# GAP-LAB-CUHK-SZ/gaustudio

Measured on NVIDIA B200. Metric: views/sec fwd+bwd @1M Gaussians/1080p, higher is better.
Workload: dtype f32

## Files before the change

gaustudio_b200/_C.py:

```python
import ctypes as C
import threading

import torch

from . import _lib

_pipeline = threading.local()


def set_pipelined(enabled, slack=1.25, fixed_capacity=None):
    _pipeline.enabled = bool(enabled)
    _pipeline.fixed = int(fixed_capacity) if fixed_capacity else 0
    _pipeline.slack = float(slack)
    _pipeline.hw = {}
    _pipeline.pending = []
    _pipeline.ring = None
    _pipeline.slot = 0
    _pipeline.rmax = None


def _pl():
    if not hasattr(_pipeline, "enabled"):
        set_pipelined(False)
    return _pipeline
# ... 229 lines not shown
        radii = radii.contiguous()
        with _on_device(dev):
            stream = torch.cuda.current_stream(dev)
            rc = L.gsr_backward(P, int(degree), M, int(R), _ptr(background), W, H, _ptr(means3D), _ptr(sh),
                                _ptr(colors), _ptr(scales), float(scale_modifier), _ptr(rotations),
                                _ptr(cov3D_precomp), _ptr(viewmatrix), _ptr(projmatrix), _ptr(campos), float(tan_fovx),
                                float(tan_fovy), _ptr(radii), _ptr(geomBuffer), _ptr(binningBuffer),
                                _ptr(imageBuffer), _ptr(gc), _ptr(gd), _ptr(gm), _ptr(go), _ptr(dL_dmeans2D), None,
                                _ptr(dL_dopacity), _ptr(dL_dcolors), None, _ptr(dL_dmeans3D), _ptr(dL_dcov3D),
                                _ptr(dL_dsh), _ptr(dL_dscales), _ptr(dL_drotations), int(bool(debug)),
                                stream.cuda_stream)
        if rc < 0:
            raise RuntimeError("gsr_backward failed: " + _lib.last_error())
    return dL_dmeans2D, dL_dcolors, dL_dopacity, dL_dmeans3D, dL_dcov3D, dL_dsh, dL_dscales, dL_drotations


def rasterize_gaussians_fused_backward(background, means3D, radii, f_dc, f_rest, opacity_logits, log_scales,
                                       raw_rotations, scale_modifier, viewmatrix, projmatrix, tan_fovx, tan_fovy,
                                       dL_dout_color, dL_dout_depth, dL_dout_median_depth, dL_dout_final_opacity,
                                       degree, campos, geomBuffer, R, binningBuffer, imageBuffer, debug):
    L = _lib.lib()
    dev = means3D.device
    P = means3D.size(0)
    H, W = dL_dout_color.size(1), dL_dout_color.size(2)
    fopt = dict(dtype=torch.float32, device=dev)
    f_dc, f_rest = _f32(f_dc, dev, "f_dc"), _f32(f_rest, dev, "f_rest")
    M = 1 + (f_rest.numel() // (3 * P) if f_rest.numel() else 0)
    d_m3 = torch.empty(P, 3, **fopt); d_m2 = torch.empty(P, 3, **fopt); d_op = torch.empty_like(opacity_logits)
    d_dc = torch.empty_like(f_dc); d_rest = torch.empty_like(f_rest); d_sc = torch.empty(P, 3, **fopt)
    d_rot = torch.empty(P, 4, **fopt); d_col = torch.empty(P, 3, **fopt); d_cov = torch.empty(P, 6, **fopt)
    means3D = _f32(means3D, dev, "means3D"); opacity_logits = _f32(opacity_logits, dev, "opacity")
    log_scales = _f32(log_scales, dev, "scales"); raw_rotations = _f32(raw_rotations, dev, "rotations")
    viewmatrix = _f32(viewmatrix, dev, "viewmatrix"); projmatrix = _f32(projmatrix, dev, "projmatrix")
    campos = _f32(campos, dev, "campos"); background = _f32(_bg_on(background, dev), dev, "bg")
    gc = _f32(dL_dout_color, dev, "dL_dout_color"); gd = _f32(dL_dout_depth, dev, "dL_dout_depth")
    gm = _f32(dL_dout_median_depth, dev, "dL_dout_median_depth"); go = _f32(dL_dout_final_opacity, dev, "dL_dout_opacity")
    with _on_device(dev):
        stream = torch.cuda.current_stream(dev)
        rc = L.gsr_backward_fused(P, int(degree), M, int(R), _ptr(background), W, H, _ptr(means3D), _ptr(f_dc),
                                  _ptr(f_rest), _ptr(opacity_logits), _ptr(log_scales), float(scale_modifier),
                                  _ptr(raw_rotations), _ptr(viewmatrix), _ptr(projmatrix), _ptr(campos), float(tan_fovx),
                                  float(tan_fovy), _ptr(radii), _ptr(geomBuffer), _ptr(binningBuffer), _ptr(imageBuffer),
                                  _ptr(gc), _ptr(gd), _ptr(gm), _ptr(go), _ptr(d_m2), _ptr(d_op), _ptr(d_col), _ptr(d_m3),
                                  _ptr(d_cov), _ptr(d_dc), _ptr(d_rest), _ptr(d_sc), _ptr(d_rot), int(bool(debug)),
                                  stream.cuda_stream)
    if rc < 0:
        raise RuntimeError("gsr_backward_fused failed: " + _lib.last_error())
    return d_m2, d_op, d_m3, d_dc, d_rest, d_sc, d_rot


def mark_visible(means3D, viewmatrix, projmatrix):
    L = _lib.lib()
    dev = means3D.device
    P = means3D.size(0)
    present = torch.zeros(P, dtype=torch.bool, device=dev)
    if P != 0:
        means3D = _f32(means3D, dev, "means3D")
        viewmatrix = _f32(viewmatrix, dev, "viewmatrix"); projmatrix = _f32(projmatrix, dev, "projmatrix")
        with torch.cuda.device(dev):
            rc = L.gsr_mark_visible(P, _ptr(means3D), _ptr(viewmatrix), _ptr(projmatrix), present.data_ptr(),
                                    torch.cuda.current_stream(dev).cuda_stream)
        if rc < 0:
            raise RuntimeError("gsr_mark_visible failed: " + _lib.last_error())
    return present


def debug_export(P, W, H, R, geomBuffer, binningBuffer, imageBuffer):
# ... 23 lines not shown
```

gaustudio_b200/csrc/gsr_api.cu:

```cuda
#include "../../include/gsr.h"
#include "gsr_internal.cuh"
#include <cmath>

#include <cstdio>
#include <cstdlib>
#include <atomic>
#include <cstring>
#include <mutex>
#include <string>
#include <vector>

#include <cuda.h>
#include <nvtx3/nvToolsExt.h>

namespace gsr {

namespace {
thread_local std::string g_err;

inline size_t align_up(size_t v, size_t a) { return (v + a - 1) / a * a; }

template <typename T> inline void take(char*& p, T*& out, size_t count) {
  p = reinterpret_cast<char*>(align_up(reinterpret_cast<size_t>(p), 256));
  out = reinterpret_cast<T*>(p);
// ... 187 lines not shown
  int dev = -1;
  bool ready(int d) {
    if (dev == d && counts && ev) return true;
    if (ev) { cudaEventDestroy(ev); ev = nullptr; }
    if (!counts && cudaHostAlloc(reinterpret_cast<void**>(&counts), 16, cudaHostAllocDefault) != cudaSuccess) { counts = nullptr; cudaGetLastError(); return false; }
    if (cudaEventCreateWithFlags(&ev, cudaEventDisableTiming) != cudaSuccess) { ev = nullptr; cudaGetLastError(); return false; }
    dev = d;
    return true;
  }
};
thread_local SpecHost t_spec;
inline long long spec_capacity(long long binned) { return binned + binned / 4 + 4096; }

__global__ void k_set_capacity(ImageHeader* h, unsigned long long cap) {
  h->capacity = cap;
  h->overflow = 0;
  h->num_big = 0;
  h->ticket[0] = 0;
  h->ticket[1] = 0;
}

__global__ void k_depth2normal(const float* __restrict__ depth, int W, int H, float ifx, float ify, float ox, float oy,
                               float dmin, float dmax, const float* __restrict__ rot, float* __restrict__ out) {
  const int u = blockIdx.x * blockDim.x + threadIdx.x, v = blockIdx.y * blockDim.y + threadIdx.y;
  if (u >= W || v >= H) return;
  float* o = out + ((size_t)v * W + u) * 3;
  float n0 = -1.f, n1 = -1.f, n2 = -1.f, c0, c1, c2;
  if (cross_normal(depth, u, v, W, H, ifx, ify, ox, oy, dmin, dmax, c0, c1, c2)) {
    if (rot) {
      n0 = c0 * rot[0] + c1 * rot[3] + c2 * rot[6];
      n1 = c0 * rot[1] + c1 * rot[4] + c2 * rot[7];
      n2 = c0 * rot[2] + c1 * rot[5] + c2 * rot[8];
    } else {
      n0 = c0; n1 = c1; n2 = c2;
    }
  }
  o[0] = n0; o[1] = n1; o[2] = n2;
}

__global__ void k_depth2point(const float* __restrict__ depth, int W, int H, float ifx, float ify, float ox, float oy,
                              const float* __restrict__ c2w, float* __restrict__ out) {
  const int u = blockIdx.x * blockDim.x + threadIdx.x, v = blockIdx.y * blockDim.y + threadIdx.y;
  if (u >= W || v >= H) return;
  const float z = depth[(size_t)v * W + u];
  const float uz = __fmul_rn(__fmul_rn(__fdiv_rn((float)u, (float)(W - 1)), (float)(W - 1)), z);
  const float vz = __fmul_rn(__fmul_rn(__fdiv_rn((float)v, (float)(H - 1)), (float)(H - 1)), z);
  float x = __fadd_rn(__fmul_rn(uz, ifx), __fmul_rn(z, ox));
  float y = __fadd_rn(__fmul_rn(vz, ify), __fmul_rn(z, oy));
  float zz = z;
  if (c2w) {
    const float wx = c2w[0] * x + c2w[1] * y + c2w[2] * z + c2w[3];
// ... 17 lines not shown
  if (depths) depths[i] = q1.z;
  if (rgb) { rgb[3 * i] = q1.w; rgb[3 * i + 1] = q2.x; rgb[3 * i + 2] = q2.y; }
  if (cov3D) for (int k = 0; k < 6; k++) cov3D[6 * i + k] = vis ? g.cov3D[6 * i + k] : 0.f;
  if (tiles_touched) tiles_touched[i] = g.tiles_touched[i];
  if (clamped) { const unsigned char c = vis ? g.clamped[i] : 0; clamped[3 * i] = c & 1; clamped[3 * i + 1] = (c >> 1) & 1; clamped[3 * i + 2] = (c >> 2) & 1; }
}
__global__ void k_export_list(long long R, const ImageHeader* hdr, BinView b, uint32_t* point_list) {
  const long long i = (long long)blockIdx.x * blockDim.x + threadIdx.x;
  const long long binned = (long long)min(hdr->num_rendered, hdr->capacity);
  if (i < R) point_list[i] = i < binned ? b.point_list[i] : 0xffffffffu;
}
__global__ void k_export_image(int N, int T, ImageView im, uint32_t* ranges, uint32_t* n_contrib, float* final_T) {
  const int i = blockIdx.x * blockDim.x + threadIdx.x;
  if (i < N) {
    if (n_contrib) n_contrib[i] = im.n_contrib[i];
    if (final_T) final_T[i] = im.final_T[i];
  }
  if (i < T && ranges) { ranges[2 * i] = im.tile_range[i].x; ranges[2 * i + 1] = im.tile_range[i].y; }
}
}

void launch_depth2normal(const float* depth, int W, int H, float fx, float fy, float cx, float cy, float dmin,
                         float dmax, const float* rot, float* out, cudaStream_t st) {
  dim3 blk(32, 8), grd((W + 31) / 32, (H + 7) / 8);
  launch_high_priority(k_depth2normal, grd, blk, 0, st, depth, W, H, 1.0f / fx, 1.0f / fy, -cx / fx, -cy / fy, dmin, dmax, rot, out);
}

void launch_depth2point(const float* depth, int W, int H, float fx, float fy, float cx, float cy, const float* c2w,
                        float* out, cudaStream_t st) {
  dim3 blk(32, 8), grd((W + 31) / 32, (H + 7) / 8);
  k_depth2point<<<grd, blk, 0, st>>>(depth, W, H, 1.0f / fx, 1.0f / fy, -cx / fx, -cy / fy, c2w, out);
}

void launch_debug_export(int P, int W, int H, long long R, GeomView g, BinView b, ImageView im,
                         uint32_t* point_list, uint32_t* ranges, uint32_t* n_contrib, float* final_T,
                         float* means2D, float* conic_opacity, float* depths, float* rgb, float* cov3D,
                         uint32_t* tiles_touched, unsigned char* clamped, cudaStream_t st) {
  if (P > 0) k_export_geom<<<(P + 255) / 256, 256, 0, st>>>(P, g, means2D, conic_opacity, depths, rgb, cov3D, tiles_touched, clamped);
  if (R > 0 && point_list) k_export_list<<<(unsigned)((R + 255) / 256), 256, 0, st>>>(R, im.hdr, b, point_list);
  const int N = W * H, T = ((W + TILE_X - 1) / TILE_X) * ((H + TILE_Y - 1) / TILE_Y);
  k_export_image<<<(max(N, T) + 255) / 256, 256, 0, st>>>(N, T, im, ranges, n_contrib, final_T);
}

}

using namespace gsr;

// ... 103 lines not shown
    if (r_host) *r_host = counts[0];
    cap = counts[0];
    ret = counts[1];
    if (!dbg && cudaGetDevice(&dev) == cudaSuccess) hint_put(dev, P, width, height, cap);
  }
  if (!second_half(cap)) return -1;
  return ret;
}

static int backward_impl(int fused, const float* f_dc, const float* f_rest, const float* opacities_raw, float* dL_df_dc, float* dL_df_rest, int P, int D, int M, int64_t R, const float* background, int width, int height,
                 const float* means3D, const float* shs, const float* colors_precomp, const float* scales,
                 float scale_modifier, const float* rotations, const float* cov3D_precomp, const float* viewmatrix,
                 const float* projmatrix, const float* campos, float tan_fovx, float tan_fovy, const int* radii,
                 char* geom_buffer, char* binning_buffer, char* image_buffer, const float* dL_dpix,
                 const float* dL_dpix_depth, const float* dL_dpix_median_depth, const float* dL_dpix_final_opacity,
                 float* dL_dmean2D, float* dL_dconic, float* dL_dopacity, float* dL_dcolor, float* dL_ddepth,
                 float* dL_dmean3D, float* dL_dcov3D, float* dL_dsh, float* dL_dscale, float* dL_drot, int debug,
                 void* stream) {
  cudaStream_t st = (cudaStream_t)stream;
  const bool dbg = debug != 0;
  if (P <= 0) return 0;
  if (!geom_buffer || !image_buffer || (!binning_buffer && R > 0)) { g_err = "gsr_backward: missing state buffers"; return -1; }
  if (!background) { g_err = "gsr_backward: background must be a device pointer (backward.cu:586 reads it)"; return -1; }
  const int gx = (width + TILE_X - 1) / TILE_X, gy = (height + TILE_Y - 1) / TILE_Y;
  GeomView g = carve_geom(aligned_base(geom_buffer), P);
  ImageView im = carve_image(aligned_base(image_buffer), width, height);
  BinView b = carve_binning(aligned_base(binning_buffer), R);
  if (radii == nullptr) radii = g.radii;

  if (!check(cudaMemsetAsync(g.grad, 0, sizeof(float) * GRAD_F * (size_t)P, st), "memset grad")) return -1;
  if (R > 0) {
    { Prof pf(5, st); launch_render_bwd(width, height, gx, gy, background, im, b, g, dL_dpix, dL_dpix_depth, dL_dpix_median_depth,
                      dL_dpix_final_opacity, st); }
    if (!stage_ok(dbg, st, "render_bwd")) return -1;
  }
  BwdArgs a;
  a.P = P; a.D = D; a.M = M; a.W = width; a.H = height;
  a.means3D = means3D; a.shs = shs; a.colors_precomp = colors_precomp; a.scales = scales; a.rotations = rotations;
  a.cov3D_precomp = cov3D_precomp; a.view = viewmatrix; a.proj = projmatrix; a.campos = campos;
  a.scale_modifier = scale_modifier; a.tan_fovx = tan_fovx; a.tan_fovy = tan_fovy;
  a.focal_y = height / (2.0f * tan_fovy);
  a.focal_x = width / (2.0f * tan_fovx);
  a.radii = radii;
  a.dL_dmean2D = dL_dmean2D; a.dL_dconic = dL_dconic; a.dL_dopacity = dL_dopacity; a.dL_dcolor = dL_dcolor;
  a.dL_ddepth = dL_ddepth; a.dL_dmean3D = dL_dmean3D; a.dL_dcov3D = dL_dcov3D; a.dL_dsh = dL_dsh;
  a.dL_dscale = dL_dscale; a.dL_drot = dL_drot;
// ... 216 lines not shown
```

gaustudio_b200/csrc/gsr_extract.cu:

```cuda
#include "gsr_internal.cuh"
#include "../../include/gsr.h"
#include <cmath>

namespace gsr {

__device__ __forceinline__ unsigned f2key(float f) {
  const unsigned b = __float_as_uint(f);
  return (b & 0x80000000u) ? ~b : (b | 0x80000000u);
}
__device__ __forceinline__ float key2f(unsigned k) {
  return __uint_as_float((k & 0x80000000u) ? (k & 0x7fffffffu) : ~k);
}

__global__ void k_minmax_init(unsigned* scratch) { scratch[0] = 0xffffffffu; scratch[1] = 0u; }

__global__ void k_dilate_minmax(const float* __restrict__ depth, const unsigned char* __restrict__ mask, int W, int H,
                                int r, unsigned char* __restrict__ out_mask, unsigned* __restrict__ scratch) {
  const int u = blockIdx.x * blockDim.x + threadIdx.x, v = blockIdx.y * blockDim.y + threadIdx.y;
  unsigned kmin = 0xffffffffu, kmax = 0u;
  if (u < W && v < H) {
    bool ok = true;
    for (int dy = -r; dy <= r; dy++) {
      const int y = v + dy;
      if (y < 0 || y >= H) continue;
// ... 43 lines not shown
      for (int dx = -r; dx <= r; dx++) {
        const float ws = sk.w[(dy + r) * dd + dx + r];
        if (ws == 0.0f) continue;
        const int x = reflect101(u + dx, W);
        const size_t q = (size_t)y * W + x;
        const float dq = depth[q];
        const float nb = (new_mask[q] && dq == dq) ? __fdiv_rn(__fsub_rn(dq, vmin), rng) : 0.0f;
        const float diff = fabsf(nb - c);
        const float w = ws * expf(diff * diff * gauss_color);
        sum = fmaf(nb, w, sum);
        wsum += w;
      }
    }
    res = __fadd_rn(__fmul_rn(__fdiv_rn(sum, wsum), rng), vmin);
  }
  out[pix] = res;
}

__global__ void k_extract_normals(const float* __restrict__ depth, const unsigned char* __restrict__ fg,
                                  const float* __restrict__ opacity, const float* __restrict__ median_depth, int W,
                                  int H, float ifx, float ify, float ox, float oy, const float* __restrict__ rot,
                                  float depth_limit, float opacity_min, float* __restrict__ cam_normals,
                                  float* __restrict__ neg_world, unsigned char* __restrict__ valid) {
  const int u = blockIdx.x * blockDim.x + threadIdx.x, v = blockIdx.y * blockDim.y + threadIdx.y;
  if (u >= W || v >= H) return;
  const size_t pix = (size_t)v * W + u;
  float c0, c1, c2;
  if (!fg[pix] || !cross_normal(depth, u, v, W, H, ifx, ify, ox, oy, 1e-3f, 100000.0f, c0, c1, c2)) c0 = c1 = c2 = -1.f;
  const float w0 = c0 * rot[0] + c1 * rot[3] + c2 * rot[6];
  const float w1 = c0 * rot[1] + c1 * rot[4] + c2 * rot[7];
  const float w2 = c0 * rot[2] + c1 * rot[5] + c2 * rot[8];
  const bool ok = (w0 + w1 + w2 > -3.0f) && median_depth[pix] < depth_limit && opacity[pix] > opacity_min;
  if (cam_normals) { cam_normals[3 * pix] = c0; cam_normals[3 * pix + 1] = c1; cam_normals[3 * pix + 2] = c2; }
  neg_world[3 * pix] = -w0; neg_world[3 * pix + 1] = -w1; neg_world[3 * pix + 2] = -w2;
  valid[pix] = ok;
}

__device__ __forceinline__ void red_add(float* p, float v) {
  asm volatile("red.global.add.f32 [%0], %1;" ::"l"(p), "f"(v) : "memory");
}

__global__ void k_fusion_pass(long long n, const long long* __restrict__ ids, const float* __restrict__ normals,
                              const float* __restrict__ conf, int P, const float* __restrict__ xyz, float tx, float ty,
                              float tz, const float* __restrict__ mean, float thresh, float* __restrict__ sum_normals,
                              float* __restrict__ sum_weights, unsigned char* __restrict__ touched) {
  const long long i = (long long)blockIdx.x * blockDim.x + threadIdx.x;
  if (i >= n) return;
  const long long id = ids[i];
  if (id < 0 || id >= P) return;
  const float nx = normals[3 * i], ny = normals[3 * i + 1], nz = normals[3 * i + 2];
  const float vx = tx - xyz[3 * id], vy = ty - xyz[3 * id + 1], vz = tz - xyz[3 * id + 2];
// ... 14 lines not shown
__global__ void k_fusion_mean(int P, const float* __restrict__ sum_normals, const float* __restrict__ sum_weights,
                              float* __restrict__ mean) {
  const int i = blockIdx.x * blockDim.x + threadIdx.x;
  if (i >= P) return;
  const float w = sum_weights[i];
  const float x = sum_normals[3 * i] / w, y = sum_normals[3 * i + 1] / w, z = sum_normals[3 * i + 2] / w;
  const float len = fmaxf(sqrtf(x * x + y * y + z * z), 1e-12f);
  mean[3 * i] = x / len; mean[3 * i + 1] = y / len; mean[3 * i + 2] = z / len;
}

void launch_masked_bilateral(const float* depth, const unsigned char* mask, int W, int H, int r, float gauss_color,
                             const SpaceKernel& sk, float* out_depth, unsigned char* out_mask, unsigned* scratch,
                             cudaStream_t st) {
  dim3 blk(32, 8), grd((W + 31) / 32, (H + 7) / 8);
  k_minmax_init<<<1, 1, 0, st>>>(scratch);
  k_dilate_minmax<<<grd, blk, 0, st>>>(depth, mask, W, H, r, out_mask, scratch);
  k_bilateral<<<grd, blk, 0, st>>>(depth, out_mask, W, H, r, gauss_color, sk, scratch, out_depth);
}

void launch_extract_normals(const float* depth, const unsigned char* fg, const float* opacity, const float* median_depth,
                            int W, int H, float fx, float fy, float cx, float cy, const float* rot, float depth_limit,
                            float opacity_min, float* cam_normals, float* neg_world, unsigned char* valid,
                            cudaStream_t st) {
  dim3 blk(32, 8), grd((W + 31) / 32, (H + 7) / 8);
  k_extract_normals<<<grd, blk, 0, st>>>(depth, fg, opacity, median_depth, W, H, 1.0f / fx, 1.0f / fy, -cx / fx, -cy / fy,
                                         rot, depth_limit, opacity_min, cam_normals, neg_world, valid);
}

void launch_fusion_pass(long long n, const long long* ids, const float* normals, const float* conf, int P,
                        const float* xyz, float tx, float ty, float tz, const float* mean, float thresh,
                        float* sum_normals, float* sum_weights, unsigned char* touched, cudaStream_t st) {
  if (n <= 0) return;
  k_fusion_pass<<<(unsigned)((n + 255) / 256), 256, 0, st>>>(n, ids, normals, conf, P, xyz, tx, ty, tz, mean, thresh,
                                                             sum_normals, sum_weights, touched);
}

void launch_fusion_mean(int P, const float* sum_normals, const float* sum_weights, float* mean, cudaStream_t st) {
  k_fusion_mean<<<(P + 255) / 256, 256, 0, st>>>(P, sum_normals, sum_weights, mean);
}

}

namespace gsr {
constexpr int KNN_MAX_K = 16;
template <int K>
__global__ void __launch_bounds__(128) k_knn_grid(int n, const float* __restrict__ pts, const int* __restrict__ cell_start,
                                                  const float* __restrict__ grid, int* __restrict__ out_index,
// ... 157 lines not shown
```

gaustudio_b200/csrc/gsr_internal.cuh:

```cuda
#pragma once

#include <cuda_runtime.h>
#include <stdint.h>
#include <stddef.h>

namespace gsr {

constexpr int TILE_X = 16;
constexpr int TILE_Y = 16;
constexpr int TILE_PIX = TILE_X * TILE_Y;
constexpr int SUBBINS = 16;

constexpr int SPLAT_F4 = 3;
constexpr int SPLAT_BYTES = 48;
constexpr int GRAD_F = 12;

struct ImageHeader {
  unsigned long long num_rendered;
  unsigned long long num_rect;
  unsigned long long capacity;
  unsigned int overflow;
  unsigned int num_big;
  unsigned int ticket[2];
  unsigned int pad[6];
// ... 134 lines not shown
  return r;
}
__device__ __forceinline__ bool may_touch(const CullRec& r, float rx0, float ry0, float rx1, float ry1) {
  if (!r.live) return false;
  const float dxlo = r.gx - rx1, dxhi = r.gx - rx0, dylo = r.gy - ry1, dyhi = r.gy - ry0;
  const bool inx = dxlo <= 0.f && dxhi >= 0.f, iny = dylo <= 0.f && dyhi >= 0.f;
  if ((inx && iny) || r.odd) return true;
  float qmin = 3.0e38f;
  if (!inx) {
    const float dxe = dxlo > 0.f ? dxlo : dxhi;
    const float dys = fminf(fmaxf(r.nBiC * dxe, dylo), dyhi);
    qmin = r.A * dxe * dxe + 2.f * r.B * dxe * dys + r.C * dys * dys;
  }
  if (!iny) {
    const float dye = dylo > 0.f ? dylo : dyhi;
    const float dxs = fminf(fmaxf(r.nBiA * dye, dxlo), dxhi);
    qmin = fminf(qmin, r.A * dxs * dxs + 2.f * r.B * dxs * dye + r.C * dye * dye);
  }
  const float mx = fmaxf(fabsf(dxlo), fabsf(dxhi)), my = fmaxf(fabsf(dylo), fabsf(dyhi));
  const float S = r.A * mx * mx + r.C * my * my + 2.f * fabsf(r.B) * mx * my;
  return !(qmin > r.tau + 1e-5f * S + 1e-3f);
}

__device__ __forceinline__ bool cross_normal(const float* __restrict__ depth, int u, int v, int W, int H, float ifx,
                                             float ify, float ox, float oy, float dmin, float dmax, float& c0,
                                             float& c1, float& c2) {
  if (!(u > 0 && v > 0 && u < W - 1 && v < H - 1)) return false;
  auto point = [&](int uu, int vv, float& x, float& y, float& z) {
    z = depth[(size_t)vv * W + uu];
    const float uz = __fmul_rn(__fmul_rn(__fdiv_rn((float)uu, (float)(W - 1)), (float)(W - 1)), z);
    const float vz = __fmul_rn(__fmul_rn(__fdiv_rn((float)vv, (float)(H - 1)), (float)(H - 1)), z);
    x = __fadd_rn(__fmul_rn(uz, ifx), __fmul_rn(z, ox));
    y = __fadd_rn(__fmul_rn(vz, ify), __fmul_rn(z, oy));
  };
  float cx, cy, cz, tx, ty, tz, bx, by, bz, lx, ly, lz, rx, ry, rz;
  point(u, v, cx, cy, cz); point(u, v - 1, tx, ty, tz); point(u, v + 1, bx, by, bz);
  point(u - 1, v, lx, ly, lz); point(u + 1, v, rx, ry, rz);
  auto ok = [&](float z) { return z > dmin && z < dmax; };
  if (!(ok(cz) && ok(tz) && ok(bz) && ok(lz) && ok(rz))) return false;
  const float ax = tx - bx, ay = ty - by, az = tz - bz, hx = lx - rx, hy = ly - ry, hz = lz - rz;
  c0 = -(__fmul_rn(ay, hz) - __fmul_rn(az, hy));
  c1 = -(__fmul_rn(az, hx) - __fmul_rn(ax, hz));
  c2 = -(__fmul_rn(ax, hy) - __fmul_rn(ay, hx));
  const float len = fmaxf(sqrtf(c0 * c0 + c1 * c1 + c2 * c2), 1e-12f);
  c0 /= len; c1 /= len; c2 /= len;
  return true;
}

struct SpaceKernel { float w[225]; };
void launch_masked_bilateral(const float* depth, const unsigned char* mask, int W, int H, int r, float gauss_color,
                             const SpaceKernel& sk, float* out_depth, unsigned char* out_mask, unsigned* scratch,
                             cudaStream_t st);
void launch_extract_normals(const float* depth, const unsigned char* fg, const float* opacity, const float* median_depth,
                            int W, int H, float fx, float fy, float cx, float cy, const float* rot, float depth_limit,
                            float opacity_min, float* cam_normals, float* neg_world, unsigned char* valid,
                            cudaStream_t st);
void launch_fusion_pass(long long n, const long long* ids, const float* normals, const float* conf, int P,
                        const float* xyz, float tx, float ty, float tz, const float* mean, float thresh,
                        float* sum_normals, float* sum_weights, unsigned char* touched, cudaStream_t st);
void launch_fusion_mean(int P, const float* sum_normals, const float* sum_weights, float* mean, cudaStream_t st);
// ... 10 lines not shown
```

gaustudio_b200/csrc/gsr_preprocess.cu:

```cuda
#include "gsr_internal.cuh"

#include <cstdio>

namespace gsr {

namespace {

__device__ const float kC0 = 0.28209479177387814f;
__device__ const float kC1 = 0.4886025119029199f;
__device__ const float kC2[5] = {1.0925484305920792f, -1.0925484305920792f, 0.31539156525252005f,
                                 -1.0925484305920792f, 0.5462742152960396f};
__device__ const float kC3[7] = {-0.5900435899266435f, 2.890611442640554f, -0.4570457994644658f,
                                 0.3731763325901154f,  -0.4570457994644658f, 1.445305721320277f,
                                 -0.5900435899266435f};

struct V3 { float x, y, z; };

#ifndef GSR_PRE_THREADS
#define GSR_PRE_THREADS 128
#endif
constexpr int PRE_THREADS = GSR_PRE_THREADS;
constexpr int SH_ROW = 52;
__device__ __forceinline__ unsigned smem_addr(const void* p) { return (unsigned)__cvta_generic_to_shared(p); }
__device__ __forceinline__ void bulk_load(void* dst, const void* src, unsigned bytes, unsigned long long* bar) {
// ... 349 lines not shown
      bar_init_expect(&sh_bar, b_dc + b_rest);
      bulk_load(sh_stage, a.f_dc + (size_t)blockIdx.x * PRE_THREADS * 3, b_dc, &sh_bar);
      bulk_load(sh_stage + PRE_THREADS * 3, a.f_rest + (size_t)blockIdx.x * PRE_THREADS * rest_row, b_rest, &sh_bar);
    }
    __syncthreads();
  }
  const bool rows = a.sh_rows && (blockIdx.x + 1) * PRE_THREADS <= a.P;
  if (rows) {
    if (threadIdx.x == 0) {
      asm volatile("mbarrier.init.shared::cta.b64 [%0], %1;" ::"r"(smem_addr(&sh_bar)), "r"(PRE_THREADS) : "memory");
      asm volatile("fence.mbarrier_init.release.cluster;" ::: "memory");
    }
    __syncthreads();
    row_load(sh_stage + threadIdx.x * SH_ROW, a.shs + (size_t)idx * 48, 192, &sh_bar);
  }
  if (!bulk && !rows && idx >= a.P) return;
  const bool vis = a.radii[idx] > 0;
  const float4* ga = reinterpret_cast<const float4*>(g.grad + (size_t)idx * GRAD_F);
  float4 g0 = make_float4(0, 0, 0, 0), g1 = g0, g2 = g0;
  if (vis) { g0 = ga[0]; g1 = ga[1]; g2 = ga[2]; }
  const float dL_dcolor[3] = {g0.x, g0.y, g0.z};
  const float dL_ddepth = g0.w, dL_dopac = g1.x;
  float dm2x = 0.f, dm2y = 0.f;
  if (vis) {
    const float4 s0 = g.splat[(size_t)idx * SPLAT_F4], s1 = g.splat[(size_t)idx * SPLAT_F4 + 1];
    const float cA = s0.z, cB = s0.w, cC = s1.x;
    dm2x = -(cA * g1.y + cB * g1.z) * (float)(0.5 * a.W);
    dm2y = -(cC * g1.z + cB * g1.y) * (float)(0.5 * a.H);
  }
  const float dcon_x = -0.5f * g1.w, dcon_y = -0.5f * g2.x, dcon_w = -0.5f * g2.y;

  a.dL_dmean2D[3 * idx] = dm2x; a.dL_dmean2D[3 * idx + 1] = dm2y; a.dL_dmean2D[3 * idx + 2] = 0.f;
  if (a.fused) {
    const float so = act_sigmoid(a.opacities_raw[idx]);
    a.dL_dopacity[idx] = dL_dopac * so * (1.0f - so);
  } else {
    a.dL_dopacity[idx] = dL_dopac;
  }
  a.dL_dcolor[3 * idx] = dL_dcolor[0]; a.dL_dcolor[3 * idx + 1] = dL_dcolor[1]; a.dL_dcolor[3 * idx + 2] = dL_dcolor[2];
  if (a.dL_dconic) reinterpret_cast<float4*>(a.dL_dconic)[idx] = make_float4(dcon_x, dcon_y, 0.f, dcon_w);
  if (a.dL_ddepth) a.dL_ddepth[idx] = dL_ddepth;

  float dmean[3] = {0.f, 0.f, 0.f};
  float dcv[6] = {0.f, 0.f, 0.f, 0.f, 0.f, 0.f};
  float dsc[3] = {0.f, 0.f, 0.f};
  float4 dq = make_float4(0.f, 0.f, 0.f, 0.f);
  float* dsh0 = a.fused ? a.dL_df_dc + (size_t)idx * 3 : (a.dL_dsh ? a.dL_dsh + (size_t)idx * M * 3 : nullptr);
  float* dshr = a.fused ? a.dL_df_rest + (size_t)idx * (M - 1) * 3 : (dsh0 ? dsh0 + 3 : nullptr);
  if (bulk) {
    bar_wait0(&sh_bar);
    dsh0 = sh_stage + threadIdx.x * 3;
    dshr = sh_stage + PRE_THREADS * 3 + threadIdx.x * rest_row;
  } else if (rows) {
    bar_wait0(&sh_bar);
    dsh0 = sh_stage + threadIdx.x * SH_ROW;
    dshr = dsh0 + 3;
  }
  auto dsh_zero = [&](int from) {
    if (!dsh0) return;
    if (from == 0) { dsh0[0] = 0.f; dsh0[1] = 0.f; dsh0[2] = 0.f; from = 1; }
    for (int k = from; k < M; k++) { dshr[3 * (k - 1)] = 0.f; dshr[3 * (k - 1) + 1] = 0.f; dshr[3 * (k - 1) + 2] = 0.f; }
  };
  const bool have_sh = a.fused || a.shs != nullptr;

  if (vis) {
    const V3 mean = {a.means3D[3 * idx], a.means3D[3 * idx + 1], a.means3D[3 * idx + 2]};
    const float* cov3D = a.cov3D_precomp ? a.cov3D_precomp + 6 * idx : g.cov3D + 6 * idx;
    float c3[6];
#pragma unroll
    for (int k = 0; k < 6; k++) c3[k] = cov3D[k];
    Cov2D cc;
    cov2d(mean, a.focal_x, a.focal_y, a.tan_fovx, a.tan_fovy, c3, a.view, cc);
    const float ca = cc.cov.m[0][0], cb = cc.cov.m[0][1], cd = cc.cov.m[1][1];
    const float det = ca * cd - cb * cb;
    const float kreg = 1.0f / ((det * det) + 0.0000001f);
    float S00 = 0.f, S01 = 0.f, S11 = 0.f;
    if (kreg != 0) {
      const float h0 = cd * dcon_x - cb * dcon_y, h1 = cd * dcon_y - cb * dcon_w;
      const float h2 = ca * dcon_y - cb * dcon_x, h3 = ca * dcon_w - cb * dcon_y;
      S00 = -kreg * (h0 * cd - h1 * cb);
      S01 = -kreg * (h1 * ca - h0 * cb);
      S11 = -kreg * (h3 * ca - h2 * cb);
    }
    float A2[2][3], Vs[3][3], Wr[3][3];
#pragma unroll
    for (int k = 0; k < 3; k++) {
      A2[0][k] = cc.T.m[0][k]; A2[1][k] = cc.T.m[1][k];
#pragma unroll
      for (int j = 0; j < 3; j++) { Vs[k][j] = cc.Vrk.m[k][j]; Wr[k][j] = a.view[4 * j + k]; }
    }
    float SA[2][3];
#pragma unroll
    for (int k = 0; k < 3; k++) { SA[0][k] = S00 * A2[0][k] + S01 * A2[1][k]; SA[1][k] = S01 * A2[0][k] + S11 * A2[1][k]; }
    if (kreg != 0) {
      auto dV = [&](int k, int l) { return A2[0][k] * SA[0][l] + A2[1][k] * SA[1][l]; };
// ... 67 lines not shown
          emit(8, kC2[4] * (xx - yy), kC2[4] * 2.f * x, kC2[4] * 2.f * -y, 0.f);
          used = 9;
          if (a.D > 2) {
            emit(9, kC3[0] * y * (3.f * xx - yy), kC3[0] * 3.f * 2.f * xy, kC3[0] * 3.f * (xx - yy), 0.f);
            emit(10, kC3[1] * xy * z, kC3[1] * yz, kC3[1] * xz, kC3[1] * xy);
            emit(11, kC3[2] * y * (4.f * zz - xx - yy), kC3[2] * -2.f * xy, kC3[2] * (-3.f * yy + 4.f * zz - xx), kC3[2] * 4.f * 2.f * yz);
            emit(12, kC3[3] * z * (2.f * zz - 3.f * xx - 3.f * yy), kC3[3] * -3.f * 2.f * xz, kC3[3] * -3.f * 2.f * yz, kC3[3] * 3.f * (2.f * zz - xx - yy));
            emit(13, kC3[4] * x * (4.f * zz - xx - yy), kC3[4] * (-3.f * xx + 4.f * zz - yy), kC3[4] * -2.f * xy, kC3[4] * 4.f * 2.f * xz);
            emit(14, kC3[5] * z * (xx - yy), kC3[5] * 2.f * xz, kC3[5] * -2.f * yz, kC3[5] * (xx - yy));
            emit(15, kC3[6] * x * (xx - 3.f * yy), kC3[6] * 3.f * (xx - yy), kC3[6] * -3.f * 2.f * xy, 0.f);
            used = 16;
          }
        }
      }
      dsh_zero(used);
      const float sum2 = ox * ox + oy * oy + oz * oz;
      const float invsum32 = 1.0f / sqrt(sum2 * sum2 * sum2);
      dmean[0] += ((+sum2 - ox * ox) * ddx - oy * ox * ddy - oz * ox * ddz) * invsum32;
      dmean[1] += (-ox * oy * ddx + (sum2 - oy * oy) * ddy - oz * oy * ddz) * invsum32;
      dmean[2] += (-ox * oz * ddx - oy * oz * ddy + (sum2 - oz * oz) * ddz) * invsum32;
    }

    if (a.scales) {
      float4 q = reinterpret_cast<const float4*>(a.rotations)[idx];
      float as0 = a.scales[3 * idx], as1 = a.scales[3 * idx + 1], as2 = a.scales[3 * idx + 2];
      if (a.fused) { q = act_normalize(q); as0 = expf(as0); as1 = expf(as1); as2 = expf(as2); }
      const float r = q.x, x = q.y, y = q.z, z = q.w;
      const float Rq[3][3] = {{1.f - 2.f * (y * y + z * z), 2.f * (x * y - r * z), 2.f * (x * z + r * y)},
                              {2.f * (x * y + r * z), 1.f - 2.f * (x * x + z * z), 2.f * (y * z - r * x)},
                              {2.f * (x * z - r * y), 2.f * (y * z + r * x), 1.f - 2.f * (x * x + y * y)}};
      const float sv[3] = {a.scale_modifier * as0, a.scale_modifier * as1, a.scale_modifier * as2};
      const float dSg[3][3] = {{dcv[0], 0.5f * dcv[1], 0.5f * dcv[2]},
                               {0.5f * dcv[1], dcv[3], 0.5f * dcv[4]},
                               {0.5f * dcv[2], 0.5f * dcv[4], dcv[5]}};
      float dR[3][3];
#pragma unroll
      for (int i = 0; i < 3; i++) {
        float acc = 0.f;
#pragma unroll
        for (int rr = 0; rr < 3; rr++) {
          const float dN = 2.f * sv[i] * (dSg[rr][0] * Rq[0][i] + dSg[rr][1] * Rq[1][i] + dSg[rr][2] * Rq[2][i]);
          acc += dN * Rq[rr][i];
          dR[rr][i] = dN * sv[i];
        }
        dsc[i] = acc;
      }
      dq.x = 2.f * (z * (dR[1][0] - dR[0][1]) + y * (dR[0][2] - dR[2][0]) + x * (dR[2][1] - dR[1][2]));
      dq.y = 2.f * (y * (dR[0][1] + dR[1][0]) + z * (dR[0][2] + dR[2][0]) + r * (dR[2][1] - dR[1][2])) - 4.f * x * (dR[1][1] + dR[2][2]);
      dq.z = 2.f * (x * (dR[0][1] + dR[1][0]) + r * (dR[0][2] - dR[2][0]) + z * (dR[1][2] + dR[2][1])) - 4.f * y * (dR[0][0] + dR[2][2]);
      dq.w = 2.f * (r * (dR[1][0] - dR[0][1]) + x * (dR[0][2] + dR[2][0]) + y * (dR[1][2] + dR[2][1])) - 4.f * z * (dR[0][0] + dR[1][1]);
      if (a.fused) {
        dsc[0] *= as0; dsc[1] *= as1; dsc[2] *= as2;
        float inv_n;
        act_normalize(reinterpret_cast<const float4*>(a.rotations)[idx], &inv_n);
        const float dot = q.x * dq.x + q.y * dq.y + q.z * dq.z + q.w * dq.w;
        dq = make_float4((dq.x - q.x * dot) * inv_n, (dq.y - q.y * dot) * inv_n, (dq.z - q.z * dot) * inv_n,
                         (dq.w - q.w * dot) * inv_n);
      }
    }
  } else {
    dsh_zero(0);
  }
  if (vis && !have_sh) dsh_zero(0);
  a.dL_dmean3D[3 * idx] = dmean[0]; a.dL_dmean3D[3 * idx + 1] = dmean[1]; a.dL_dmean3D[3 * idx + 2] = dmean[2];
#pragma unroll
  for (int k = 0; k < 6; k++) a.dL_dcov3D[6 * idx + k] = dcv[k];
  a.dL_dscale[3 * idx] = dsc[0]; a.dL_dscale[3 * idx + 1] = dsc[1]; a.dL_dscale[3 * idx + 2] = dsc[2];
  reinterpret_cast<float4*>(a.dL_drot)[idx] = dq;
  if (bulk) {
    asm volatile("fence.proxy.async.shared::cta;" ::: "memory");
    __syncthreads();
    if (threadIdx.x == 0) {
      bulk_store(a.dL_df_dc + (size_t)blockIdx.x * PRE_THREADS * 3, sh_stage, PRE_THREADS * 3 * 4);
      bulk_store(a.dL_df_rest + (size_t)blockIdx.x * PRE_THREADS * rest_row, sh_stage + PRE_THREADS * 3,
                 PRE_THREADS * rest_row * 4);
      asm volatile("cp.async.bulk.commit_group;" ::: "memory");
      asm volatile("cp.async.bulk.wait_group.read 0;" ::: "memory");
    }
  } else if (rows) {
    asm volatile("fence.proxy.async.shared::cta;" ::: "memory");
    bulk_store(a.dL_dsh + (size_t)idx * 48, sh_stage + threadIdx.x * SH_ROW, 192);
    asm volatile("cp.async.bulk.commit_group;" ::: "memory");
    asm volatile("cp.async.bulk.wait_group.read 0;" ::: "memory");
  }
}

__global__ void k_mark_visible(int P, const float* __restrict__ means3D, const float* __restrict__ view,
                               unsigned char* __restrict__ present) {
  const int idx = blockIdx.x * blockDim.x + threadIdx.x;
// ... 32 lines not shown
```

gaustudio_b200/csrc/gsr_render.cu:

```cuda
#include "gsr_internal.cuh"
#include <cstdlib>
#include <cstring>
#include <cuda.h>

namespace gsr {

namespace {

#ifndef GSR_RB
#define GSR_RB 128
#endif
#ifndef GSR_NSTAGE
#define GSR_NSTAGE 4
#endif
constexpr int RB = GSR_RB;
constexpr int NSTAGE = GSR_NSTAGE;
static_assert(RB % 32 == 0 && RB >= 32 && NSTAGE >= 1, "ring geometry");
constexpr int STAGE_F4 = RB * SPLAT_F4;
constexpr int NBLK = TILE_PIX / 32;
constexpr unsigned FULL = 0xffffffffu;

__device__ __forceinline__ unsigned smem_u32(const void* p) { return (unsigned)__cvta_generic_to_shared(p); }

__device__ __forceinline__ void mbar_init(unsigned long long* bar, unsigned count) {
// ... 282 lines not shown
        __syncwarp();
      }
      const int hi = nmax - b * RB, lo = max(0, hi - RB);
      stage_gather(ring.buf[s], splat, ids + lo, hi - lo, lane, &ring.full[s]);
    }
    return;
  }

  const size_t HW = (size_t)W * H;
  const int lx = lane & 7, ly = lane >> 3;
  const int bx0 = tx * TILE_X, by0 = ty * TILE_Y;
  float T[NSUB], Q[NSUB], g0[NSUB], g1[NSUB], g2[NSUB], gD[NSUB], gO[NSUB], gM[NSUB];
  int lastc[NSUB], maxs[NSUB];
  int warp_max = 0;
#pragma unroll
  for (int s = 0; s < NSUB; s++) {
    const int px = bx0 + blk_kx<NSUB>(warp, s) * 8 + lx, py = by0 + blk_ky<NSUB>(warp, s) * 4 + ly;
    const bool inside = px < W && py < H;
    const size_t pid = (size_t)py * W + px;
    T[s] = inside ? im.final_T[pid] : 0.f;
    lastc[s] = inside ? (int)im.n_contrib[pid] : 0;
    g0[s] = g1[s] = g2[s] = gD[s] = gO[s] = gM[s] = 0.f;
    if (inside) {
      g0[s] = dL_dpix[pid]; g1[s] = dL_dpix[HW + pid]; g2[s] = dL_dpix[2 * HW + pid];
      gD[s] = dL_ddepthpix[pid];
      gO[s] = dL_dopacpix[pid];
      gM[s] = dL_dmedpix[pid];
    }
    float bg_dot = 0.f;
    bg_dot += bg[0] * g0[s]; bg_dot += bg[1] * g1[s]; bg_dot += bg[2] * g2[s];
    Q[s] = T[s] * bg_dot;
    maxs[s] = (int)__reduce_max_sync(FULL, (unsigned)lastc[s]);
    warp_max = max(warp_max, maxs[s]);
  }
  const bool pub = (lane & 1) == 0 && ((lane & 2) == 0 || (lane & 12) == 0);
  const int slot = ((lane & 16) ? 5 : 0) + ((lane & 2) ? 4 : ((lane & 4) ? 2 : 0) + ((lane & 8) ? 1 : 0));
  unsigned lanebits = (unsigned)lane | (pub ? 32u : 0u);
  float* gslot = grad + slot;
  asm volatile("" : "+r"(lanebits), "+l"(gslot));

  for (int b = 0; b < nb; b++) {
    const int st = b % NSTAGE;
    mbar_wait(&ring.full[st], (unsigned)((b / NSTAGE) & 1));
    const int hi = nmax - b * RB, lo = max(0, hi - RB), cnt = hi - lo;
    const float4* sb = ring.buf[st];
    if (lo < warp_max) {
      for (int base = 0; base < cnt; base += 32) {
        const int j = cnt - 1 - (base + lane);
        unsigned m[NSUB];
        {
// ... 147 lines not shown
```

gaustudio_b200/rasterizer.py:

```python
from typing import NamedTuple

import torch
import torch.nn as nn

from . import _C


def cpu_deep_copy_tuple(input_tuple):
    return tuple(item.cpu().clone() if isinstance(item, torch.Tensor) else item for item in input_tuple)


def rasterize_gaussians(means3D, means2D, sh, colors_precomp, opacities, scales, rotations, cov3Ds_precomp,
                        raster_settings):
    return _RasterizeGaussians.apply(means3D, means2D, sh, colors_precomp, opacities, scales, rotations,
                                     cov3Ds_precomp, raster_settings)


class _RasterizeGaussians(torch.autograd.Function):
    @staticmethod
    def forward(ctx, means3D, means2D, sh, colors_precomp, opacities, scales, rotations, cov3Ds_precomp,
                raster_settings):
        rs = raster_settings
        args = (rs.bg, means3D, colors_precomp, opacities, scales, rotations, rs.scale_modifier, cov3Ds_precomp,
                rs.viewmatrix, rs.projmatrix, rs.tanfovx, rs.tanfovy, rs.image_height, rs.image_width, sh,
# ... 36 lines not shown
        else:
            out = _C.rasterize_gaussians_backward(*args)
        (grad_means2D, grad_colors_precomp, grad_opacities, grad_means3D, grad_cov3Ds_precomp, grad_sh, grad_scales,
         grad_rotations) = out
        return (grad_means3D, grad_means2D, grad_sh, grad_colors_precomp, grad_opacities, grad_scales, grad_rotations,
                grad_cov3Ds_precomp, None)


class _RasterizeGaussiansFused(torch.autograd.Function):

    @staticmethod
    def forward(ctx, means3D, means2D, f_dc, f_rest, opacity_logits, log_scales, raw_rotations, raster_settings):
        rs = raster_settings
        e = torch.Tensor([])
        out = _C.rasterize_gaussians(rs.bg, means3D, e, opacity_logits, log_scales, raw_rotations, rs.scale_modifier, e,
                                     rs.viewmatrix, rs.projmatrix, rs.tanfovx, rs.tanfovy, rs.image_height,
                                     rs.image_width, e, rs.sh_degree, rs.campos, rs.prefiltered, rs.debug,
                                     _fused=(f_dc, f_rest))
        num_rendered, color, depth, median_depth, final_opacity, radii, geomBuffer, binningBuffer, imgBuffer = out
        ctx.raster_settings, ctx.num_rendered = rs, num_rendered
        ctx.save_for_backward(means3D, f_dc, f_rest, opacity_logits, log_scales, raw_rotations, radii, geomBuffer,
                              binningBuffer, imgBuffer)
        ctx.mark_non_differentiable(radii)
        return color, radii, depth, median_depth, final_opacity

    @staticmethod
    def backward(ctx, grad_out_color, grad_radii, grad_depth, grad_median_depth, grad_final_opacity):
        rs = ctx.raster_settings
        means3D, f_dc, f_rest, opac, scales, rots, radii, geomBuffer, binningBuffer, imgBuffer = ctx.saved_tensors
        d_m2, d_op, d_m3, d_dc, d_rest, d_sc, d_rot = _C.rasterize_gaussians_fused_backward(
            rs.bg, means3D, radii, f_dc, f_rest, opac, scales, rots, rs.scale_modifier, rs.viewmatrix, rs.projmatrix,
            rs.tanfovx, rs.tanfovy, grad_out_color, grad_depth, grad_median_depth, grad_final_opacity, rs.sh_degree,
            rs.campos, geomBuffer, ctx.num_rendered, binningBuffer, imgBuffer, rs.debug)
        return d_m3, d_m2, d_dc, d_rest, d_op, d_sc, d_rot, None


def rasterize_gaussians_fused(means3D, means2D, f_dc, f_rest, opacity_logits, log_scales, raw_rotations,
                              raster_settings):
    return _RasterizeGaussiansFused.apply(means3D, means2D, f_dc, f_rest, opacity_logits, log_scales, raw_rotations,
                                          raster_settings)


class GaussianRasterizationSettings(NamedTuple):
    image_height: int
    image_width: int
    tanfovx: float
# ... 43 lines not shown
```

Measured before the change: 1062.

## Skip unused gradient outputs, recompute cov3D in backward, precompute grid coords

After: 1084, median of 6. +2.1%, better.

```diff
diff --git a/gaustudio_b200/_C.py b/gaustudio_b200/_C.py
--- a/gaustudio_b200/_C.py
+++ b/gaustudio_b200/_C.py
@@ -275,13 +275,14 @@
     L = _lib.lib()
     dev = means3D.device
     P = means3D.size(0)
-    H, W = dL_dout_color.size(1), dL_dout_color.size(2)
+    grads = (dL_dout_color, dL_dout_depth, dL_dout_median_depth, dL_dout_final_opacity)
+    H, W = next(g for g in grads if g is not None).shape[-2:]
     fopt = dict(dtype=torch.float32, device=dev)
     f_dc, f_rest = _f32(f_dc, dev, "f_dc"), _f32(f_rest, dev, "f_rest")
     M = 1 + (f_rest.numel() // (3 * P) if f_rest.numel() else 0)
     d_m3 = torch.empty(P, 3, **fopt); d_m2 = torch.empty(P, 3, **fopt); d_op = torch.empty_like(opacity_logits)
     d_dc = torch.empty_like(f_dc); d_rest = torch.empty_like(f_rest); d_sc = torch.empty(P, 3, **fopt)
-    d_rot = torch.empty(P, 4, **fopt); d_col = torch.empty(P, 3, **fopt); d_cov = torch.empty(P, 6, **fopt)
+    d_rot = torch.empty(P, 4, **fopt)
     means3D = _f32(means3D, dev, "means3D"); opacity_logits = _f32(opacity_logits, dev, "opacity")
     log_scales = _f32(log_scales, dev, "scales"); raw_rotations = _f32(raw_rotations, dev, "rotations")
     viewmatrix = _f32(viewmatrix, dev, "viewmatrix"); projmatrix = _f32(projmatrix, dev, "projmatrix")
@@ -294,8 +295,8 @@
                                   _ptr(f_rest), _ptr(opacity_logits), _ptr(log_scales), float(scale_modifier),
                                   _ptr(raw_rotations), _ptr(viewmatrix), _ptr(projmatrix), _ptr(campos), float(tan_fovx),
                                   float(tan_fovy), _ptr(radii), _ptr(geomBuffer), _ptr(binningBuffer), _ptr(imageBuffer),
-                                  _ptr(gc), _ptr(gd), _ptr(gm), _ptr(go), _ptr(d_m2), _ptr(d_op), _ptr(d_col), _ptr(d_m3),
-                                  _ptr(d_cov), _ptr(d_dc), _ptr(d_rest), _ptr(d_sc), _ptr(d_rot), int(bool(debug)),
+                                  _ptr(gc), _ptr(gd), _ptr(gm), _ptr(go), _ptr(d_m2), _ptr(d_op), None, _ptr(d_m3),
+                                  None, _ptr(d_dc), _ptr(d_rest), _ptr(d_sc), _ptr(d_rot), int(bool(debug)),
                                   stream.cuda_stream)
     if rc < 0:
         raise RuntimeError("gsr_backward_fused failed: " + _lib.last_error())
diff --git a/gaustudio_b200/csrc/gsr_api.cu b/gaustudio_b200/csrc/gsr_api.cu
--- a/gaustudio_b200/csrc/gsr_api.cu
+++ b/gaustudio_b200/csrc/gsr_api.cu
@@ -233,11 +233,13 @@
 
 __global__ void k_depth2normal(const float* __restrict__ depth, int W, int H, float ifx, float ify, float ox, float oy,
                                float dmin, float dmax, const float* __restrict__ rot, float* __restrict__ out) {
-  const int u = blockIdx.x * blockDim.x + threadIdx.x, v = blockIdx.y * blockDim.y + threadIdx.y;
+  __shared__ GridCoords gc;
+  grid_coords_fill(gc, W, H);
+  const int u = blockIdx.x * PIX_BX + threadIdx.x, v = blockIdx.y * PIX_BY + threadIdx.y;
   if (u >= W || v >= H) return;
   float* o = out + ((size_t)v * W + u) * 3;
   float n0 = -1.f, n1 = -1.f, n2 = -1.f, c0, c1, c2;
-  if (cross_normal(depth, u, v, W, H, ifx, ify, ox, oy, dmin, dmax, c0, c1, c2)) {
+  if (cross_normal(depth, u, v, W, H, ifx, ify, ox, oy, dmin, dmax, gc, c0, c1, c2)) {
     if (rot) {
       n0 = c0 * rot[0] + c1 * rot[3] + c2 * rot[6];
       n1 = c0 * rot[1] + c1 * rot[4] + c2 * rot[7];
@@ -301,7 +303,7 @@
 
 void launch_depth2normal(const float* depth, int W, int H, float fx, float fy, float cx, float cy, float dmin,
                          float dmax, const float* rot, float* out, cudaStream_t st) {
-  dim3 blk(32, 8), grd((W + 31) / 32, (H + 7) / 8);
+  dim3 blk(PIX_BX, PIX_BY), grd((W + PIX_BX - 1) / PIX_BX, (H + PIX_BY - 1) / PIX_BY);
   launch_high_priority(k_depth2normal, grd, blk, 0, st, depth, W, H, 1.0f / fx, 1.0f / fy, -cx / fx, -cy / fy, dmin, dmax, rot, out);
 }
 
@@ -451,6 +453,7 @@
   if (P <= 0) return 0;
   if (!geom_buffer || !image_buffer || (!binning_buffer && R > 0)) { g_err = "gsr_backward: missing state buffers"; return -1; }
   if (!background) { g_err = "gsr_backward: background must be a device pointer (backward.cu:586 reads it)"; return -1; }
+  if (cov3D_precomp == nullptr && (scales == nullptr || rotations == nullptr)) { g_err = "gsr_backward: need scales+rotations or cov3D_precomp"; return -1; }
   const int gx = (width + TILE_X - 1) / TILE_X, gy = (height + TILE_Y - 1) / TILE_Y;
   GeomView g = carve_geom(aligned_base(geom_buffer), P);
   ImageView im = carve_image(aligned_base(image_buffer), width, height);
diff --git a/gaustudio_b200/csrc/gsr_extract.cu b/gaustudio_b200/csrc/gsr_extract.cu
--- a/gaustudio_b200/csrc/gsr_extract.cu
+++ b/gaustudio_b200/csrc/gsr_extract.cu
@@ -89,11 +89,13 @@
                                   int H, float ifx, float ify, float ox, float oy, const float* __restrict__ rot,
                                   float depth_limit, float opacity_min, float* __restrict__ cam_normals,
                                   float* __restrict__ neg_world, unsigned char* __restrict__ valid) {
-  const int u = blockIdx.x * blockDim.x + threadIdx.x, v = blockIdx.y * blockDim.y + threadIdx.y;
+  __shared__ GridCoords gc;
+  grid_coords_fill(gc, W, H);
+  const int u = blockIdx.x * PIX_BX + threadIdx.x, v = blockIdx.y * PIX_BY + threadIdx.y;
   if (u >= W || v >= H) return;
   const size_t pix = (size_t)v * W + u;
   float c0, c1, c2;
-  if (!fg[pix] || !cross_normal(depth, u, v, W, H, ifx, ify, ox, oy, 1e-3f, 100000.0f, c0, c1, c2)) c0 = c1 = c2 = -1.f;
+  if (!fg[pix] || !cross_normal(depth, u, v, W, H, ifx, ify, ox, oy, 1e-3f, 100000.0f, gc, c0, c1, c2)) c0 = c1 = c2 = -1.f;
   const float w0 = c0 * rot[0] + c1 * rot[3] + c2 * rot[6];
   const float w1 = c0 * rot[1] + c1 * rot[4] + c2 * rot[7];
   const float w2 = c0 * rot[2] + c1 * rot[5] + c2 * rot[8];
@@ -154,7 +156,7 @@
                             int W, int H, float fx, float fy, float cx, float cy, const float* rot, float depth_limit,
                             float opacity_min, float* cam_normals, float* neg_world, unsigned char* valid,
                             cudaStream_t st) {
-  dim3 blk(32, 8), grd((W + 31) / 32, (H + 7) / 8);
+  dim3 blk(PIX_BX, PIX_BY), grd((W + PIX_BX - 1) / PIX_BX, (H + PIX_BY - 1) / PIX_BY);
   k_extract_normals<<<grd, blk, 0, st>>>(depth, fg, opacity, median_depth, W, H, 1.0f / fx, 1.0f / fy, -cx / fx, -cy / fy,
                                          rot, depth_limit, opacity_min, cam_normals, neg_world, valid);
 }
diff --git a/gaustudio_b200/csrc/gsr_internal.cuh b/gaustudio_b200/csrc/gsr_internal.cuh
--- a/gaustudio_b200/csrc/gsr_internal.cuh
+++ b/gaustudio_b200/csrc/gsr_internal.cuh
@@ -180,20 +180,35 @@
   return !(qmin > r.tau + 1e-5f * S + 1e-3f);
 }
 
+__device__ __forceinline__ float grid_coord(int i, int n) {
+  return __fmul_rn(__fdiv_rn((float)i, (float)(n - 1)), (float)(n - 1));
+}
+constexpr int PIX_BX = 32, PIX_BY = 8;
+struct GridCoords { float u[PIX_BX + 2], v[PIX_BY + 2]; };
+__device__ __forceinline__ void grid_coords_fill(GridCoords& s, int W, int H) {
+  const int t = threadIdx.y * PIX_BX + threadIdx.x;
+  const int u0 = blockIdx.x * PIX_BX - 1, v0 = blockIdx.y * PIX_BY - 1;
+  if (t < PIX_BX + 2) s.u[t] = grid_coord(u0 + t, W);
+  else if (t >= 64 && t < 64 + PIX_BY + 2) s.v[t - 64] = grid_coord(v0 + t - 64, H);
+  __syncthreads();
+}
+
 __device__ __forceinline__ bool cross_normal(const float* __restrict__ depth, int u, int v, int W, int H, float ifx,
-                                             float ify, float ox, float oy, float dmin, float dmax, float& c0,
-                                             float& c1, float& c2) {
+                                             float ify, float ox, float oy, float dmin, float dmax,
+                                             const GridCoords& gc, float& c0, float& c1, float& c2) {
   if (!(u > 0 && v > 0 && u < W - 1 && v < H - 1)) return false;
-  auto point = [&](int uu, int vv, float& x, float& y, float& z) {
-    z = depth[(size_t)vv * W + uu];
-    const float uz = __fmul_rn(__fmul_rn(__fdiv_rn((float)uu, (float)(W - 1)), (float)(W - 1)), z);
-    const float vz = __fmul_rn(__fmul_rn(__fdiv_rn((float)vv, (float)(H - 1)), (float)(H - 1)), z);
+  const float* cu = gc.u + (threadIdx.x + 1);
+  const float* cv = gc.v + (threadIdx.y + 1);
+  auto point = [&](int du, int dv, float& x, float& y, float& z) {
+    z = depth[(size_t)(v + dv) * W + (u + du)];
+    const float uz = __fmul_rn(cu[du], z);
+    const float vz = __fmul_rn(cv[dv], z);
     x = __fadd_rn(__fmul_rn(uz, ifx), __fmul_rn(z, ox));
     y = __fadd_rn(__fmul_rn(vz, ify), __fmul_rn(z, oy));
   };
   float cx, cy, cz, tx, ty, tz, bx, by, bz, lx, ly, lz, rx, ry, rz;
-  point(u, v, cx, cy, cz); point(u, v - 1, tx, ty, tz); point(u, v + 1, bx, by, bz);
-  point(u - 1, v, lx, ly, lz); point(u + 1, v, rx, ry, rz);
+  point(0, 0, cx, cy, cz); point(0, -1, tx, ty, tz); point(0, 1, bx, by, bz);
+  point(-1, 0, lx, ly, lz); point(1, 0, rx, ry, rz);
   auto ok = [&](float z) { return z > dmin && z < dmax; };
   if (!(ok(cz) && ok(tz) && ok(bz) && ok(lz) && ok(rz))) return false;
   const float ax = tx - bx, ay = ty - by, az = tz - bz, hx = lx - rx, hy = ly - ry, hz = lz - rz;
diff --git a/gaustudio_b200/csrc/gsr_preprocess.cu b/gaustudio_b200/csrc/gsr_preprocess.cu
--- a/gaustudio_b200/csrc/gsr_preprocess.cu
+++ b/gaustudio_b200/csrc/gsr_preprocess.cu
@@ -395,22 +395,17 @@
   const float dL_dcolor[3] = {g0.x, g0.y, g0.z};
   const float dL_ddepth = g0.w, dL_dopac = g1.x;
   float dm2x = 0.f, dm2y = 0.f;
-  if (vis) {
-    const float4 s0 = g.splat[(size_t)idx * SPLAT_F4], s1 = g.splat[(size_t)idx * SPLAT_F4 + 1];
-    const float cA = s0.z, cB = s0.w, cC = s1.x;
-    dm2x = -(cA * g1.y + cB * g1.z) * (float)(0.5 * a.W);
-    dm2y = -(cC * g1.z + cB * g1.y) * (float)(0.5 * a.H);
-  }
   const float dcon_x = -0.5f * g1.w, dcon_y = -0.5f * g2.x, dcon_w = -0.5f * g2.y;
 
-  a.dL_dmean2D[3 * idx] = dm2x; a.dL_dmean2D[3 * idx + 1] = dm2y; a.dL_dmean2D[3 * idx + 2] = 0.f;
   if (a.fused) {
     const float so = act_sigmoid(a.opacities_raw[idx]);
     a.dL_dopacity[idx] = dL_dopac * so * (1.0f - so);
   } else {
     a.dL_dopacity[idx] = dL_dopac;
   }
-  a.dL_dcolor[3 * idx] = dL_dcolor[0]; a.dL_dcolor[3 * idx + 1] = dL_dcolor[1]; a.dL_dcolor[3 * idx + 2] = dL_dcolor[2];
+  if (a.dL_dcolor) {
+    a.dL_dcolor[3 * idx] = dL_dcolor[0]; a.dL_dcolor[3 * idx + 1] = dL_dcolor[1]; a.dL_dcolor[3 * idx + 2] = dL_dcolor[2];
+  }
   if (a.dL_dconic) reinterpret_cast<float4*>(a.dL_dconic)[idx] = make_float4(dcon_x, dcon_y, 0.f, dcon_w);
   if (a.dL_ddepth) a.dL_ddepth[idx] = dL_ddepth;
 
@@ -438,12 +433,33 @@
 
   if (vis) {
     const V3 mean = {a.means3D[3 * idx], a.means3D[3 * idx + 1], a.means3D[3 * idx + 2]};
-    const float* cov3D = a.cov3D_precomp ? a.cov3D_precomp + 6 * idx : g.cov3D + 6 * idx;
+    float4 q = make_float4(0.f, 0.f, 0.f, 0.f);
+    float as0 = 0.f, as1 = 0.f, as2 = 0.f;
+    if (a.scales) {
+      q = reinterpret_cast<const float4*>(a.rotations)[idx];
+      as0 = a.scales[3 * idx]; as1 = a.scales[3 * idx + 1]; as2 = a.scales[3 * idx + 2];
+      if (a.fused) { q = act_normalize(q); as0 = expf(as0); as1 = expf(as1); as2 = expf(as2); }
+    }
     float c3[6];
-#pragma unroll
-    for (int k = 0; k < 6; k++) c3[k] = cov3D[k];
+    if (a.cov3D_precomp) {
+#pragma unroll
+      for (int k = 0; k < 6; k++) c3[k] = a.cov3D_precomp[6 * idx + k];
+    } else {
+      const float mod = a.scale_modifier;
+      const Mat3 Mm = mmul(scale_mat(mod * as0, mod * as1, mod * as2), quat_mat(q.x, q.y, q.z, q.w));
+      const Mat3 Sg = mmul(mtr(Mm), Mm);
+      c3[0] = Sg.m[0][0]; c3[1] = Sg.m[0][1]; c3[2] = Sg.m[0][2];
+      c3[3] = Sg.m[1][1]; c3[4] = Sg.m[1][2]; c3[5] = Sg.m[2][2];
+    }
     Cov2D cc;
     cov2d(mean, a.focal_x, a.focal_y, a.tan_fovx, a.tan_fovy, c3, a.view, cc);
+    {
+      const float cx = cc.cov.m[0][0], cy = cc.cov.m[0][1], cz = cc.cov.m[1][1];
+      const float det_inv = 1.f / (cx * cz - cy * cy);
+      const float cA = cz * det_inv, cB = -cy * det_inv, cC = cx * det_inv;
+      dm2x = -(cA * g1.y + cB * g1.z) * (float)(0.5 * a.W);
+      dm2y = -(cC * g1.z + cB * g1.y) * (float)(0.5 * a.H);
+    }
     const float ca = cc.cov.m[0][0], cb = cc.cov.m[0][1], cd = cc.cov.m[1][1];
     const float det = ca * cd - cb * cb;
     const float kreg = 1.0f / ((det * det) + 0.0000001f);
@@ -557,9 +573,6 @@
     }
 
     if (a.scales) {
-      float4 q = reinterpret_cast<const float4*>(a.rotations)[idx];
-      float as0 = a.scales[3 * idx], as1 = a.scales[3 * idx + 1], as2 = a.scales[3 * idx + 2];
-      if (a.fused) { q = act_normalize(q); as0 = expf(as0); as1 = expf(as1); as2 = expf(as2); }
       const float r = q.x, x = q.y, y = q.z, z = q.w;
       const float Rq[3][3] = {{1.f - 2.f * (y * y + z * z), 2.f * (x * y - r * z), 2.f * (x * z + r * y)},
                               {2.f * (x * y + r * z), 1.f - 2.f * (x * x + z * z), 2.f * (y * z - r * x)},
@@ -597,9 +610,12 @@
     dsh_zero(0);
   }
   if (vis && !have_sh) dsh_zero(0);
+  a.dL_dmean2D[3 * idx] = dm2x; a.dL_dmean2D[3 * idx + 1] = dm2y; a.dL_dmean2D[3 * idx + 2] = 0.f;
   a.dL_dmean3D[3 * idx] = dmean[0]; a.dL_dmean3D[3 * idx + 1] = dmean[1]; a.dL_dmean3D[3 * idx + 2] = dmean[2];
-#pragma unroll
-  for (int k = 0; k < 6; k++) a.dL_dcov3D[6 * idx + k] = dcv[k];
+  if (a.dL_dcov3D) {
+#pragma unroll
+    for (int k = 0; k < 6; k++) a.dL_dcov3D[6 * idx + k] = dcv[k];
+  }
   a.dL_dscale[3 * idx] = dsc[0]; a.dL_dscale[3 * idx + 1] = dsc[1]; a.dL_dscale[3 * idx + 2] = dsc[2];
   reinterpret_cast<float4*>(a.dL_drot)[idx] = dq;
   if (bulk) {
diff --git a/gaustudio_b200/csrc/gsr_render.cu b/gaustudio_b200/csrc/gsr_render.cu
--- a/gaustudio_b200/csrc/gsr_render.cu
+++ b/gaustudio_b200/csrc/gsr_render.cu
@@ -328,10 +328,10 @@
     lastc[s] = inside ? (int)im.n_contrib[pid] : 0;
     g0[s] = g1[s] = g2[s] = gD[s] = gO[s] = gM[s] = 0.f;
     if (inside) {
-      g0[s] = dL_dpix[pid]; g1[s] = dL_dpix[HW + pid]; g2[s] = dL_dpix[2 * HW + pid];
-      gD[s] = dL_ddepthpix[pid];
-      gO[s] = dL_dopacpix[pid];
-      gM[s] = dL_dmedpix[pid];
+      if (dL_dpix) { g0[s] = dL_dpix[pid]; g1[s] = dL_dpix[HW + pid]; g2[s] = dL_dpix[2 * HW + pid]; }
+      if (dL_ddepthpix) gD[s] = dL_ddepthpix[pid];
+      if (dL_dopacpix) gO[s] = dL_dopacpix[pid];
+      if (dL_dmedpix) gM[s] = dL_dmedpix[pid];
     }
     float bg_dot = 0.f;
     bg_dot += bg[0] * g0[s]; bg_dot += bg[1] * g1[s]; bg_dot += bg[2] * g2[s];
diff --git a/gaustudio_b200/rasterizer.py b/gaustudio_b200/rasterizer.py
--- a/gaustudio_b200/rasterizer.py
+++ b/gaustudio_b200/rasterizer.py
@@ -82,6 +82,7 @@
         ctx.save_for_backward(means3D, f_dc, f_rest, opacity_logits, log_scales, raw_rotations, radii, geomBuffer,
                               binningBuffer, imgBuffer)
         ctx.mark_non_differentiable(radii)
+        ctx.set_materialize_grads(False)
         return color, radii, depth, median_depth, final_opacity
 
     @staticmethod
```
